# danping/CoSLAM

Measured on AMD Instinct MI355X. Metric: frames/sec for track+local-BA loop, 8 cams 640x480 x 2000 feats (one frame = all 8 cameras), higher is better.
Workload: dtype f32 (KLT, f16 pyramid storage) + f64 (pose, BA)

## Files before the change

### coslam_amd/csrc/cs_common.h

```cpp
#pragma once

#include <hip/hip_fp16.h>
#include <hip/hip_runtime.h>

#include <cstdarg>
#include <cstdint>
#include <cstdio>
#include <cstring>

#include "../../include/coslam_hip.h"

#define CS_MAX_LEVELS 12
#define CS_WAVE 64

void cs_set_error(const char* fmt, ...);
enum { CS_DBG_BA_SYRK = 0, CS_DBG_BA_PACKED = 1, CS_DBG_BA_GRAPHS = 2, CS_DBG_MERGE_PRINT = 3, CS_DBG_COUNT = 4 };
int cs_debug_get(int which);

#define CS_HIP(call)                                                                              \
    do {                                                                                          \
        hipError_t _e = (call);                                                                   \
        if (_e != hipSuccess) {                                                                   \
            cs_set_error("%s failed: %s (%s:%d)", #call, hipGetErrorString(_e), __FILE__, __LINE__); \
            return CS_ERR_HIP;                                                                    \
        }                                                                                         \
    } while (0)

#define CS_CHECK_LAUNCH()                                                                        \
    do {                                                                                         \
        hipError_t _e = hipGetLastError();                                                       \
        if (_e != hipSuccess) {                                                                  \
            cs_set_error("kernel launch failed: %s (%s:%d)", hipGetErrorString(_e), __FILE__, __LINE__); \
            return CS_ERR_HIP;                                                                   \
        }                                                                                        \
    } while (0)

struct CsPyrLayout {
    int W, H, L;
    int w[CS_MAX_LEVELS], h[CS_MAX_LEVELS];
    int64_t off[CS_MAX_LEVELS];
    size_t texels;
};

static inline CsPyrLayout cs_make_layout(int W, int H, int L) {
    CsPyrLayout p;
    memset(&p, 0, sizeof(p));
    p.W = W;
    p.H = H;
    p.L = L;
// ... 82 lines not shown
}

__device__ __forceinline__ double cs_wave_sum_d(double v) {
    v += cs_dpp_d<0xB1, 0xf>(v);
    v += cs_dpp_d<0x4E, 0xf>(v);
    v += cs_dpp_d<0x141, 0xf>(v);
    v += cs_dpp_d<0x140, 0xf>(v);
    v += cs_dpp_d<0x142, 0xa>(v);
    v += cs_dpp_d<0x143, 0xc>(v);
    int lo = __builtin_amdgcn_readlane(__double2loint(v), 63);
    int hi = __builtin_amdgcn_readlane(__double2hiint(v), 63);
    return __hiloint2double(hi, lo);
}

__device__ __forceinline__ int cs_wave_sum_i(int v) {
    v += cs_dpp_i<0xB1, 0xf>(v);
    v += cs_dpp_i<0x4E, 0xf>(v);
    v += cs_dpp_i<0x141, 0xf>(v);
    v += cs_dpp_i<0x140, 0xf>(v);
    v += cs_dpp_i<0x142, 0xa>(v);
    v += cs_dpp_i<0x143, 0xc>(v);
    return __builtin_amdgcn_readlane(v, 63);
}

__device__ __forceinline__ double cs_shfl_xor_d(double v, int d) {
    int lo = __shfl_xor(__double2loint(v), d, 64), hi = __shfl_xor(__double2hiint(v), d, 64);
    return __hiloint2double(hi, lo);
}
__device__ __forceinline__ double cs_readlane_d(double v, int l) {
    int lo = __builtin_amdgcn_readlane(__double2loint(v), l);
    int hi = __builtin_amdgcn_readlane(__double2hiint(v), l);
    return __hiloint2double(hi, lo);
}
template <int M, int DIST>
__device__ __forceinline__ void cs_reduce_step(double* v, int lane) {
    if constexpr (DIST >= 1) {
        constexpr int H = (M + 1) / 2;
        const bool up = (lane & DIST) != 0;
#pragma unroll
        for (int t = 0; t < H; ++t) {
            const double lo = v[t];
            const double hi = (H + t < M) ? v[H + t] : 0.0;
            const double recv = cs_shfl_xor_d(up ? lo : hi, DIST);
            v[t] = (up ? hi : lo) + recv;
        }
        cs_reduce_step<H, DIST / 2>(v, lane);
    }
}
template <int N>
__device__ __forceinline__ void cs_reduce_many(double* v, int lane) {
    cs_reduce_step<N, 32>(v, lane);
}
template <int N>
__host__ __device__ constexpr int cs_reduce_index(int lane) {
    int lo = 0, end = N, m = N;
    for (int d = 32; d >= 1; d >>= 1) {
        const int h = (m + 1) / 2;
        if (lane & d) {
            lo += h;
        } else {
            end = end < lo + h ? end : lo + h;
        }
        m = h;
    }
    return lo < end ? lo : -1;
}
template <int N>
__host__ __device__ constexpr int cs_reduce_owner(int q) {
    for (int l = 0; l < 64; ++l)
        if (cs_reduce_index<N>(l) == q) return l;
    return 0;
}
template <int N>
struct CsOwnerTable {
    int lane[N];
    constexpr CsOwnerTable() : lane{} {
        for (int q = 0; q < N; ++q) lane[q] = cs_reduce_owner<N>(q);
// ... 22 lines not shown
```

### coslam_amd/csrc/klt_seq.hip

```cpp
#include <cstdlib>
#include <mutex>
#include <new>
#include <vector>

#include "klt_internal.h"

static thread_local char g_err[512] = "";
void cs_set_error(const char* fmt, ...) {
    va_list ap;
    va_start(ap, fmt);
    vsnprintf(g_err, sizeof(g_err), fmt, ap);
    va_end(ap);
}

#include <atomic>
static std::atomic<int> g_dbg[CS_DBG_COUNT] = {{-1}, {-1}, {-1}, {-1}};
int cs_debug_get(int which) { return which >= 0 && which < CS_DBG_COUNT ? g_dbg[which].load(std::memory_order_relaxed) : -1; }

extern "C" {

int cs_version(void) { return 100; }
const char* cs_last_error(void) { return g_err; }
int cs_debug_set(const char* key, int value) {
    static const char* names[CS_DBG_COUNT] = {"ba_syrk", "ba_packed", "ba_graphs", "merge_print"};
    for (int k = 0; k < CS_DBG_COUNT; ++k)
        if (key && !strcmp(key, names[k])) {
            g_dbg[k].store(value, std::memory_order_relaxed);
            return CS_OK;
        }
    cs_set_error("cs_debug_set: unknown switch (ba_syrk, ba_packed, ba_graphs, merge_print)");
    return CS_ERR_INVALID;
}


int cs_device_count(void) {
    int n = 0;
    if (hipGetDeviceCount(&n) != hipSuccess) return 0;
    return n;
}

void* cs_stream_create_cu_range(int device, int first_cu, int n_cus) {
    hipDeviceProp_t prop;
    if (hipSetDevice(device) != hipSuccess || hipGetDeviceProperties(&prop, device) != hipSuccess) {
        cs_set_error("cs_stream_create_cu_range: bad device %d", device);
        return nullptr;
    }
    const int total = prop.multiProcessorCount;
    if (first_cu < 0 || n_cus <= 0 || first_cu + n_cus > total) {
        cs_set_error("cs_stream_create_cu_range: range [%d, %d) outside the %d CUs", first_cu, first_cu + n_cus, total);
        return nullptr;
    }
    std::vector<uint32_t> mask((total + 31) / 32, 0u);
    for (int c = first_cu; c < first_cu + n_cus; ++c) mask[c >> 5] |= 1u << (c & 31);
    hipStream_t s = nullptr;
    hipError_t e = hipExtStreamCreateWithCUMask(&s, (uint32_t)mask.size(), mask.data());
    if (e != hipSuccess) {
        cs_set_error("hipExtStreamCreateWithCUMask failed: %s", hipGetErrorString(e));
        return nullptr;
    }
    return (void*)s;
}

void* cs_stream_create_cu_interleaved(int device, int period, int take, int complement) {
// ... 1405 lines not shown
```

### coslam_amd/csrc/poseupdate.hip

```cpp
#include <atomic>
#include <cstdlib>
#include <vector>

#include "cs_common.h"
#include "project_dev.h"
#include "triangulate_dev.h"
#include "history_view.h"
#include "register_rows_dev.h"
#include "small_ops.h"

#pragma clang fp contract(off)

namespace {

constexpr int PU_MAX_CAMS = 16;
constexpr int PU_MAX_HIST = 512;
constexpr int PU_MAX_STORE = 1 << 16;
constexpr int PU_LPS = 8;

struct PuArgs {
    int nCams, N, nMap, cam0, nCamsRun;
    int gateBlocks, dynBlocksPerCam;
    const int* pointFeat;
    const double* R;
// ... 2589 lines not shown
    A.nMap = nMap, A.featRef = (const int4*)d_featRef, A.mapPts = d_mapPts, A.mapCov = d_mapCov, A.sigma = pixelErrVar;
    A.refine = 1, A.select = d_select, A.selectW = d_select;
    return CS_OK;
}
}

extern "C" int cs_feat_ref_advance_refine_dev(cs_track_history* h, void* hip_stream, const cs_poseupdate_cam* cams, int nMap, const int* d_pointFeat,
                                              int curFrame, cs_feat_ref* d_featRef, unsigned char* d_refStatic, int* d_counts, const int* d_list,
                                              int nList, int advanceAll, unsigned char* d_select, int clearSelect, double* d_mapPts,
                                              double* d_mapCov, double pixelErrVar) {
    const char* who = "cs_feat_ref_advance_refine_dev";
    if (!h || !cams || nMap < 1 || nList < 1 || !d_list) {
        cs_set_error("%s: bad arguments", who);
        return CS_ERR_INVALID;
    }
    ArArgs A;
    memset((void*)&A, 0, sizeof(A));
    if (const int rc = ar_fill_refine(who, A, h, cams, nMap, curFrame, d_featRef, d_select, d_mapPts, d_mapCov, pixelErrVar)) return rc;
    if (const int rc = fr_fill(who, A.F, h, cams, nMap, d_pointFeat, curFrame, d_featRef, d_refStatic, d_counts)) return rc;
    A.list = d_list, A.nList = nList, A.advAll = advanceAll ? 1 : 0;
    A.blocksA = ((advanceAll ? nMap : nList) + 255) / 256;
    CS_HIP(hipSetDevice(h->device));
    hipStream_t s = (hipStream_t)hip_stream;
    if (const int rc = hist_alive(h, nMap, s)) return rc;
    A.F.alive = h->alive;
    hist_centres(h, s);
    hipLaunchKernelGGL(k_advance_refine, dim3(A.blocksA + (nList + 3) / 4), dim3(256), 0, s, A);
    if (clearSelect) hipLaunchKernelGGL(k_clear_marks, dim3((nList + 255) / 256), dim3(256), 0, s, d_select, d_list, nList, nMap);
    CS_HIP(hipGetLastError());
    return CS_OK;
}

constexpr int RR_THREADS = 256;
struct RrArgs {
    int nRounds, W, H;
    int* lists;
    int* rvCounts;
    cs_register_pass pass;
    cs_register_cam rcam[RG_MAX_CAMS];
    MgRunCore mg;
    RvArgs rv;
    ArArgs ar;
};
static_assert(sizeof(RrArgs) <= 4096, "k_revisit_rounds: the arguments must fit the kernel-argument segment");
template <int MC>
__global__ __launch_bounds__(RR_THREADS) void k_revisit_rounds(RrArgs A) {
    extern __shared__ double rr_pose[];
    __shared__ MgMiss missList[RR_THREADS / MG_LPC];
    __shared__ int nMiss;
    __shared__ int sCnt[RR_THREADS / 64][5];
    if (rd_ld(A.rvCounts) == 0) return;
    CS_POSE_STREAM_PRIO();
    const int tid = threadIdx.x, lane = tid & 63, wave = tid >> 6, C = A.rv.nCams, cap = A.rv.cap, N = A.rv.N;
    const cs_register_pass& Q = A.pass;
    int cnt[5] = {0, 0, 0, 0, 0};
    for (int r = 0; r < A.nRounds; ++r) {
        const int listed = rd_ld(A.rvCounts + r);
        if (listed == 0) break;
        const int n = listed < cap ? listed : cap;
        const int* list = A.lists + (size_t)r * cap;
        for (int k = wave; k < n * C; k += RR_THREADS / 64) {
            const int row = k / C, c = k - row * C, p = list[row];
            if (p < 0) continue;
            const cs_register_cam& Cm = A.rcam[c];
            const size_t o = (size_t)p * C + c;
            int outSlot = -1, outFlags = 0;
            double m0 = 0, m1 = 0, var[4] = {0, 0, 0, 0}, ivar[4] = {0, 0, 0, 0}, outDist = 0;
            Proj q;
            if (rg_pair_begin(Q, Cm, o, p, A.W, A.H, q, m0, m1, var, ivar, outSlot)) {
                double dMin;
                int iMin;
                rg_pair_scan_wave(Cm, N, lane, m0, m1, ivar, dMin, iMin);
                rg_pair_finish(Q, Cm, p, N, q, m0, m1, dMin, iMin, outSlot, outFlags, outDist);
            }
            if (lane == 0) rg_pair_store(Q, o, outSlot, outFlags, outDist, m0, m1, var);
        }
        __syncthreads();
        const int nB = (n * MG_LPC + RR_THREADS - 1) / RR_THREADS;
        for (int c = 0; c < C; ++c)
            for (int bx = 0; bx < nB; ++bx) {
                mg_running_rows<RR_THREADS>(A.mg, A.ar.cam, list, cap, c, bx, rr_pose, missList, nMiss);
                __syncthreads();
            }
        {
            const bool more = r + 1 < A.nRounds;
            const RvRound Rd{list, A.rvCounts + r, more ? A.lists + (size_t)(r + 1) * cap : nullptr, more ? A.rvCounts + r + 1 : nullptr};
            if (n <= RR_THREADS) {
                rv_decide_rows<MC>(A.rv, Rd);
            } else {
                int* rowCode = (int*)(rr_pose + 12 * (size_t)A.mg.W);
                rv_decide_rows_looped<MC, RR_THREADS>(A.rv, Rd, n, rowCode, rowCode + MC * RV_MAX_ROWS);
            }
        }
        __syncthreads();
        for (int j = tid; j < n; j += RR_THREADS) {
            const int m = list[j];
            if (m >= 0 && m < A.ar.nMap && !A.ar.select[m]) fr_advance_row(A.ar.F, A.ar.cam, m, cnt);
        }
        __syncthreads();
        for (int j = wave; j < n; j += RR_THREADS / 64) {
            const int m = list[j];
            if (m >= 0 && m < A.ar.nMap && A.ar.select[m]) {
                ar_refine_row(A.ar, m, lane, cnt);
                if (lane == 0) A.ar.selectW[m] = 0;
            }
        }
        __syncthreads();
    }
    fr_fold_counts(cnt, sCnt, A.ar.F.counts);
}
template <int MC>
static int rr_dynamic_lds_limit(int device, size_t* out) {
    static std::atomic<long long> last{-1};
    const long long c = last.load(std::memory_order_acquire);
    if (c >= 0 && (int)(c >> 32) == device) {
        *out = (size_t)(c & 0xffffffffll);
// ... 24 lines not shown
    const char* who = "cs_register_revisit_rounds_dev";
    if (!h || !regCams || !cams || !pass) {
        cs_set_error("%s: bad arguments (null history, cameras or pass)", who);
        return CS_ERR_INVALID;
    }
    const int nCams = h->nCams, N = h->N;
    const cs_register_pass& q = *pass;
    if (nCams < 1 || nCams > RG_MAX_CAMS || nCams > RD_MAX_CAMS || N < 1 || W < 1 || H < 1 || !(q.maxDist > 0) || !(q.sigmaSearch >= 0) ||
        !(q.sigmaMerge >= 0) || (q.mapFlags && !(q.maxDistDynamic > 0))) {
        cs_set_error("%s: bad arguments (1..%d cameras, N >= 1, maxDist > 0; mapFlags with maxDistDynamic > 0)", who, RD_MAX_CAMS);
        return CS_ERR_INVALID;
    }
    if (!q.M || !q.cov || !q.pointFeat || !q.slot || !q.m || !q.var || !q.dist || !q.flags || q.M != d_mapPts || q.cov != d_mapCov ||
        q.pointFeat != d_pointFeat) {
        cs_set_error("%s: the pass needs every table, and its map, covariances and feature table are the ones refined", who);
        return CS_ERR_INVALID;
    }
    if (nMap < 1 || cap < 1 || cap > RV_MAX_ROWS || nRounds < 1 || nRounds > 8 || kinds < 1 || kinds > 3 || mapBase < 0 || !(tolPix >= 0) ||
        !d_rvLists || !d_rvCounts || (long long)nCams * N > RD_FEAT || (long long)nCams * nMap * nCams > 0x7fffffffLL) {
        cs_set_error("%s: bad arguments (1..%d rows, 1..8 rounds, kinds 1..3, the rounds' lists and counts)", who, RV_MAX_ROWS);
        return CS_ERR_INVALID;
    }
    RrArgs A;
    memset((void*)&A, 0, sizeof(A));
    for (int c = 0; c < nCams; ++c) {
        const cs_register_cam& rc = regCams[c];
        if (!rc.K || !rc.R || !rc.t || !rc.xy || !rc.state || !rc.slot2map) {
            cs_set_error("%s: null pointer in search camera %d", who, c);
            return CS_ERR_INVALID;
        }
        A.rcam[c] = rc;
    }
    A.nRounds = nRounds, A.W = W, A.H = H, A.lists = d_rvLists, A.rvCounts = d_rvCounts;
    A.pass = q;
    A.pass.P = cap, A.pass.list = nullptr;
    if (const int rc = ar_fill_refine(who, A.ar, h, cams, nMap, curFrame, d_featRef, d_regOut, d_mapPts, d_mapCov, pixelErrVar)) return rc;
    if (const int rc = fr_fill(who, A.ar.F, h, cams, nMap, d_pointFeat, curFrame, d_featRef, d_refStatic, d_frefCounts)) return rc;
    if (const int rc = mg_fill_running(who, A.mg, h, cams, 0, nMap, d_mapPts, d_mapCov, q.slot, q.flags, pixelErrVar, tolPix, d_mergeCache,
                                       d_mergeable, nullptr))
        return rc;
    if (const int rc = rv_fill(who, A.rv, nCams, N, nMap, cap, mapBase, kinds, d_nextLoop, d_visitLoop, q.slot, q.flags, d_mergeable, d_mapFlags,
                               d_pointFeat, d_slot2map, d_attached, d_regOut, d_decideScratch, d_curList, d_curCount, curCap, d_rvCnt,
                               d_rvCounts + nRounds))
        return rc;
    CS_HIP(hipSetDevice(h->device));
    hipStream_t s = (hipStream_t)hip_stream;
    const int MC = nCams <= 8 ? 8 : RD_MAX_CAMS;
    const size_t lds = sizeof(double) * 12 * (size_t)A.mg.W + (cap > RR_THREADS ? sizeof(int) * (size_t)(MC + 1) * RV_MAX_ROWS : 0);
    size_t ldsMax = 0;
    if (const int rc = MC == 8 ? rr_dynamic_lds_limit<8>(h->device, &ldsMax) : rr_dynamic_lds_limit<RD_MAX_CAMS>(h->device, &ldsMax)) return rc;
    if (lds > ldsMax) {
        cs_set_error("%s: %zu B of LDS (a history window of %d frames, lists of %d rows, %d cameras) where the launch may carry %zu", who, lds,
                     A.mg.W, cap, nCams, ldsMax);
        return CS_ERR_INVALID;
    }
    if (const int rc = hist_alive(h, nMap, s)) return rc;
    A.ar.F.alive = h->alive;
    hist_centres(h, s);
    if (MC == 8)
        hipLaunchKernelGGL(k_revisit_rounds<8>, dim3(1), dim3(RR_THREADS), lds, s, A);
    else
        hipLaunchKernelGGL(k_revisit_rounds<RD_MAX_CAMS>, dim3(1), dim3(RR_THREADS), lds, s, A);
    CS_HIP(hipGetLastError());
    return CS_OK;
}

extern "C" int cs_track_history_segments(const cs_track_history* h, cs_feat_seg** d_pool, int* cap, int** d_count) {
    if (!h) {
        cs_set_error("cs_track_history_segments: null handle");
        return CS_ERR_INVALID;
    }
    if (d_pool) *d_pool = (cs_feat_seg*)h->segPool;
    if (cap) *cap = h->segCap;
    if (d_count) *d_count = h->segCount;
    return CS_OK;
}

extern "C" int cs_track_history_segment_counts(const cs_track_history* h, int* counts) {
    if (!h || !counts) {
        cs_set_error("cs_track_history_segment_counts: bad arguments");
        return CS_ERR_INVALID;
    }
    CS_HIP(hipSetDevice(h->device));
    CS_HIP(hipMemcpy(counts, h->segCount, sizeof(int) * h->nCams, hipMemcpyDeviceToHost));
    return CS_OK;
}

extern "C" int cs_track_history_load_segments(cs_track_history* h, const cs_feat_seg* segs, int n) {
    if (!h || n < 0 || n > h->segCap || (n > 0 && !segs)) {
        cs_set_error("cs_track_history_load_segments: bad arguments (at most %d segments per camera)", h ? h->segCap : 0);
        return CS_ERR_INVALID;
    }
    CS_HIP(hipSetDevice(h->device));
    std::vector<int> cnt(h->nCams, n);
    for (int c = 0; c < h->nCams && n > 0; ++c)
// ... 308 lines not shown
```

### coslam_amd/csrc/pose.hip

```cpp
#include "cs_common.h"

#pragma clang fp contract(off)

namespace {

constexpr int WS_LDS_MAX = 4096;
constexpr int SMALL_NPTS = 64;

__device__ __forceinline__ void so3_exp(const double w[3], double R[9]) {
    double theta = sqrt(w[0] * w[0] + w[1] * w[1] + w[2] * w[2]);
    if (theta == 0) {
        R[0] = 1, R[1] = 0, R[2] = 0, R[3] = 0, R[4] = 1, R[5] = 0, R[6] = 0, R[7] = 0, R[8] = 1;
        return;
    }
    double hw0 = w[0] / theta, hw1 = w[1] / theta, hw2 = w[2] / theta;
    double st, ct;
    if (theta < 0.5) {
        const double x2 = theta * theta;
        double ps = 1.0 / 355687428096000.0;
        ps = ps * x2 - 1.0 / 1307674368000.0;
        ps = ps * x2 + 1.0 / 6227020800.0;
        ps = ps * x2 - 1.0 / 39916800.0;
        ps = ps * x2 + 1.0 / 362880.0;
        ps = ps * x2 - 1.0 / 5040.0;
        ps = ps * x2 + 1.0 / 120.0;
        ps = ps * x2 - 1.0 / 6.0;
        st = theta + theta * (x2 * ps);
        double pc = 1.0 / 20922789888000.0;
        pc = pc * x2 - 1.0 / 87178291200.0;
        pc = pc * x2 + 1.0 / 479001600.0;
        pc = pc * x2 - 1.0 / 3628800.0;
        pc = pc * x2 + 1.0 / 40320.0;
        pc = pc * x2 - 1.0 / 720.0;
        pc = pc * x2 + 1.0 / 24.0;
        const double c = 1.0 - (0.5 * x2 - x2 * x2 * pc);
        ct = 1 - c;
    } else {
        st = sin(theta);
        ct = 1 - cos(theta);
    }
    double hw0hw0 = hw0 * hw0, hw0hw1 = hw0 * hw1, hw0hw2 = hw0 * hw2;
    double hw1hw1 = hw1 * hw1, hw1hw2 = hw1 * hw2, hw2hw2 = hw2 * hw2;
    R[0] = -ct * hw1hw1 - ct * hw2hw2 + 1;
    R[1] = ct * hw0hw1 - st * hw2;
    R[2] = st * hw1 + ct * hw0hw2;
    R[3] = st * hw2 + ct * hw0hw1;
    R[4] = -ct * hw0hw0 - ct * hw2hw2 + 1;
    R[5] = ct * hw1hw2 - st * hw0;
    R[6] = ct * hw0hw2 - st * hw1;
    R[7] = st * hw0 + ct * hw1hw2;
    R[8] = -ct * hw0hw0 - ct * hw1hw1 + 1;
}

__device__ __forceinline__ void mat33AB(const double* A, const double* B, double* C) {
    double T[9];
#pragma unroll
    for (int i = 0; i < 3; ++i)
#pragma unroll
        for (int j = 0; j < 3; ++j) T[3 * i + j] = A[3 * i] * B[j] + A[3 * i + 1] * B[3 + j] + A[3 * i + 2] * B[6 + j];
#pragma unroll
    for (int i = 0; i < 9; ++i) C[i] = T[i];
}

__device__ __forceinline__ void project(const double* K, const double* R, const double* t, const double* M, double* m) {
    double X = R[0] * M[0] + R[1] * M[1] + R[2] * M[2] + t[0];
    double Y = R[3] * M[0] + R[4] * M[1] + R[5] * M[2] + t[1];
    double Z = R[6] * M[0] + R[7] * M[1] + R[8] * M[2] + t[2];
    double u = K[0] * X + K[1] * Y + K[2] * Z;
    double v = K[3] * X + K[4] * Y + K[5] * Z;
    double w = K[6] * X + K[7] * Y + K[8] * Z;
    m[0] = u / w;
    m[1] = v / w;
}

__device__ __forceinline__ double cs_shfl_d(double v, int srcLane) {
    int lo = __shfl(__double2loint(v), srcLane, 64), hi = __shfl(__double2hiint(v), srcLane, 64);
    return __hiloint2double(hi, lo);
}
__device__ __forceinline__ void solve66_lanes(double m, int lane, double* param) {
    const int r = lane / 7, j = lane - 7 * r;
    const bool in = r < 6;
#pragma unroll
    for (int c = 0; c < 6; ++c) {
        double best = fabs(cs_readlane_d(m, 7 * c + c));
        int p = c;
#pragma unroll
        for (int rr = c + 1; rr < 6; ++rr) {
            const double v = fabs(cs_readlane_d(m, 7 * rr + c));
            if (v > best) best = v, p = rr;
        }
        const int srcRow = r == c ? p : (r == p ? c : r);
        const double sw = cs_shfl_d(m, in ? 7 * srcRow + j : lane);
        m = sw;
        const double d = cs_readlane_d(m, 7 * c + c);
        const double q = m / d;
        if (r == c && j > c) m = q;
        const double f = cs_shfl_d(m, in ? 7 * r + c : lane);
        const double pr = cs_shfl_d(m, in ? 7 * c + j : lane);
        const double e = m - f * pr;
        if (in && r != c && j > c) m = e;
    }
#pragma unroll
    for (int rr = 0; rr < 6; ++rr) param[rr] = cs_readlane_d(m, 7 * rr + 6);
}

__device__ __forceinline__ double tukey(double e, double tau) {
    if (e >= tau) return 0;
    e /= tau;
    e = 1 - e * e;
    return e * e;
}

struct PoseCtx {
    const double* K;
    const double* Ms;
    const double* ms;
    double* Ws;
    int npts;
    double* red;
    double pM[3], pm[2];
    double dR[3][9];
    int myEntry;
};

constexpr int NSUM = 28;
__device__ __forceinline__ int solve_entry_of_lane(int lane) {
    const int r = lane / 7, j = lane - 7 * r;
    if (r >= 6) return 27;
    if (j == 6) return 21 + r;
    const int a = r < j ? r : j, b = r < j ? j : r;
    return a * 6 - (a * (a - 1)) / 2 + (b - a);
}
template <int PB>
__device__ __forceinline__ void block_sum28(double (&v)[NSUM], double* lds , int& par, int myEntry, double& mine,
                                            double& err) {
    constexpr int NW = PB / 64;
    const int lane = threadIdx.x & 63, wv = threadIdx.x >> 6;
    cs_reduce_many<NSUM>(v, lane);
    if (NW == 1) {
        constexpr CsOwnerTable<NSUM> T{};
        int owner = 0;
#pragma unroll
        for (int q = 0; q < NSUM; ++q) owner = myEntry == q ? T.lane[q] : owner;
        mine = cs_shfl_d(v[0], owner);
        err = cs_readlane_d(v[0], T.lane[27]);
        return;
    }
    const int have = cs_reduce_index<NSUM>(lane);
    double* buf = lds + par * (NW * NSUM);
    par ^= 1;
    if (have >= 0) buf[wv * NSUM + have] = v[0];
    __syncthreads();
    double s = buf[myEntry], e = buf[27];
#pragma unroll
    for (int w = 1; w < NW; ++w) s += buf[w * NSUM + myEntry], e += buf[w * NSUM + 27];
    mine = s, err = e;
}

template <int PB>
__device__ void lm_pass(const PoseCtx& c, const double* R, const double* t, bool reweight, double tau, int& par, double& mine, double& err) {
    const double eps = 1e-8;
    const double ieps = 1e8;
    double R1[3][9];
#pragma unroll
    for (int a = 0; a < 3; ++a) mat33AB(R, c.dR[a], R1[a]);
    double acc[NSUM];
#pragma unroll
    for (int q = 0; q < NSUM; ++q) acc[q] = 0;
    for (int i = threadIdx.x; i < c.npts; i += PB) {
        double pM[3], pm[2];
        if (i < PB) {
            pM[0] = c.pM[0], pM[1] = c.pM[1], pM[2] = c.pM[2], pm[0] = c.pm[0], pm[1] = c.pm[1];
        } else {
            pM[0] = c.Ms[3 * i], pM[1] = c.Ms[3 * i + 1], pM[2] = c.Ms[3 * i + 2], pm[0] = c.ms[2 * i], pm[1] = c.ms[2 * i + 1];
        }
        double rm0[2], rm[2], J[12];
        project(c.K, R, t, pM, rm0);
        const double dx = rm0[0] - pm[0], dy = rm0[1] - pm[1];
        double w;
        if (reweight) {
            w = tukey(sqrt(dx * dx + dy * dy), tau);
            c.Ws[i] = w;
        } else {
            w = c.Ws[i];
        }
        acc[27] += (dx * dx + dy * dy) * w;
#pragma unroll
        for (int a = 0; a < 3; ++a) {
            project(c.K, R1[a], t, pM, rm);
            J[a] = (rm[0] - rm0[0]) * ieps;
            J[6 + a] = (rm[1] - rm0[1]) * ieps;
        }
#pragma unroll
        for (int a = 0; a < 3; ++a) {
            double t1[3] = {t[0], t[1], t[2]};
            t1[a] = t[a] + eps;
            project(c.K, R, t1, pM, rm);
            J[3 + a] = (rm[0] - rm0[0]) * ieps;
            J[9 + a] = (rm[1] - rm0[1]) * ieps;
        }
#pragma unroll
        for (int q = 0; q < 12; ++q) J[q] = w * J[q];
        const double r0 = (-rm0[0] + pm[0]) * w, r1 = (-rm0[1] + pm[1]) * w;
        int q = 0;
#pragma unroll
        for (int r = 0; r < 6; ++r)
#pragma unroll
            for (int cc = r; cc < 6; ++cc) acc[q++] += J[r] * J[cc] + J[6 + r] * J[6 + cc];
#pragma unroll
        for (int r = 0; r < 6; ++r) acc[21 + r] += J[r] * r0 + J[6 + r] * r1;
    }
    block_sum28<PB>(acc, c.red, par, c.myEntry, mine, err);
}

__device__ __forceinline__ void lm_solve(double mine, double lambda, double* param) {
    const int lane = threadIdx.x & 63, r = lane / 7, j = lane - 7 * r;
    solve66_lanes(r == j ? mine + lambda : mine, lane, param);
}

__device__ __forceinline__ void update_pose(const double* R, const double* t, const double* p, double* Rn, double* tn) {
    double dR[9];
    so3_exp(p, dR);
    mat33AB(R, dR, Rn);
    tn[0] = t[0] + p[3];
    tn[1] = t[1] + p[4];
    tn[2] = t[2] + p[5];
}

template <int PB>
__device__ bool weighted_lm(const PoseCtx& c, const double* R0, const double* t0, double* R_opt, double* t_opt,
                            cs_pose_option& opt, bool reweight, double tau, int& par) {
    double param[6];
    double ne, cand, err;
    opt.npts = c.npts;
    opt.lambda = opt.lambda0;
    lm_pass<PB>(c, R0, t0, reweight, tau, par, ne, err);
    opt.err0 = err;
    opt.err = opt.err0;
    double R[9], t[3], R_tmp[9], t_tmp[3];
#pragma unroll
    for (int i = 0; i < 9; ++i) R[i] = R_tmp[i] = R0[i];
#pragma unroll
    for (int i = 0; i < 3; ++i) t[i] = t_tmp[i] = t0[i];
    opt.retTypeLM = 1;
    int i = 0;
    for (; i < opt.maxIterLM; ++i) {
        lm_solve(ne, opt.lambda, param);
        update_pose(R, t, param, R_opt, t_opt);
        double p2 = param[0] * param[0] + param[1] * param[1] + param[2] * param[2] + param[3] * param[3] +
                    param[4] * param[4] + param[5] * param[5];
        if (p2 < opt.epsParamChangeLM) {
            opt.retTypeLM = 0;
            break;
        }
        lm_pass<PB>(c, R_opt, t_opt, false, tau, par, cand, err);
        if (fabs(err - opt.err) < opt.epsErrorChangeLM) {
            opt.retTypeLM = 0;
            break;
        }
        if (err <= opt.err) {
#pragma unroll
            for (int q = 0; q < 9; ++q) R[q] = R_tmp[q] = R_opt[q];
#pragma unroll
            for (int q = 0; q < 3; ++q) t[q] = t_tmp[q] = t_opt[q];
            ne = cand;
            opt.err = err;
            opt.lambda /= 10;
        } else {
            opt.lambda *= 10;
            if (opt.lambda > 1e+18) {
                opt.retTypeLM = -1;
                break;
            }
        }
    }
    if (opt.retTypeLM == -1) {
#pragma unroll
        for (int q = 0; q < 9; ++q) R_opt[q] = R_tmp[q];
#pragma unroll
        for (int q = 0; q < 3; ++q) t_opt[q] = t_tmp[q];
    }
    opt.err = err;
    opt.nIterLM = i;
    opt.verboseRW += i < opt.maxIterLM ? i + 1 : i;
    return opt.retTypeLM >= 0;
}

#if defined(CS_IC_NUM_VGPR)
#define CS_IC_ATTR __attribute__((amdgpu_num_vgpr(CS_IC_NUM_VGPR)))
#elif defined(CS_IC_WAVES_PER_EU)
#define CS_IC_ATTR __attribute__((amdgpu_waves_per_eu(CS_IC_WAVES_PER_EU, CS_IC_WAVES_PER_EU)))
#else
#define CS_IC_ATTR
#endif
template <int PB>
__global__ __launch_bounds__(PB) CS_IC_ATTR void k_intracam(int ptsStride, const double* __restrict__ Kall,
                                                 const double* __restrict__ R0all, const double* __restrict__ t0all,
                                                 const int* __restrict__ nptsAll, const double* __restrict__ prevErrs,
                                                 const double* __restrict__ MsAll, const double* __restrict__ msAll,
                                                 double tau, double* __restrict__ RoptAll, double* __restrict__ toptAll,
                                                 cs_pose_option* __restrict__ optAll, int* __restrict__ okAll,
                                                 double* __restrict__ wsScratch) {
    extern __shared__ __attribute__((aligned(16))) double smem[];
    CS_POSE_STREAM_PRIO();
    const int pb = blockIdx.x;
    constexpr int NW = PB / 64;
    double* red = smem;
    double* sK = smem + 2 * NW * NSUM;
    double* WsL = sK + 12;
    const int npts = nptsAll[pb];
    if (threadIdx.x < 9) sK[threadIdx.x] = Kall[9 * pb + threadIdx.x];
    PoseCtx c;
    c.K = sK;
    c.Ms = MsAll + (size_t)3 * ptsStride * pb;
    c.ms = msAll + (size_t)2 * ptsStride * pb;
    c.npts = npts;
    c.red = red;
    c.myEntry = solve_entry_of_lane(threadIdx.x & 63);
    c.Ws = wsScratch ? (wsScratch + (size_t)ptsStride * pb) : WsL;
#pragma unroll
    for (int a = 0; a < 3; ++a) {
        double w[3] = {0, 0, 0};
        w[a] = 1e-8;
        so3_exp(w, c.dR[a]);
    }
    if ((int)threadIdx.x < npts) {
        const int i = threadIdx.x;
        c.pM[0] = c.Ms[3 * i], c.pM[1] = c.Ms[3 * i + 1], c.pM[2] = c.Ms[3 * i + 2], c.pm[0] = c.ms[2 * i], c.pm[1] = c.ms[2 * i + 1];
    } else {
        c.pM[0] = c.pM[1] = c.pM[2] = c.pm[0] = c.pm[1] = 0;
    }
    for (int i = threadIdx.x; i < npts; i += PB)
        c.Ws[i] = prevErrs ? tukey(fabs(prevErrs[(size_t)ptsStride * pb + i]), tau) : 1.0;
    __syncthreads();

    cs_pose_option opt = optAll[pb];
    double R[9], t[3], R_opt[9], t_opt[3];
#pragma unroll
    for (int i = 0; i < 9; ++i) R[i] = R_opt[i] = R0all[9 * pb + i];
#pragma unroll
    for (int i = 0; i < 3; ++i) t[i] = t_opt[i] = t0all[3 * pb + i];
    bool ret = true;
    int k = 0, par = 0;
    opt.errRW = -1;
    opt.verboseRW = 0;
    for (; k < opt.maxIterRW; ++k) {
        if (!weighted_lm<PB>(c, R, t, R_opt, t_opt, opt, k > 0, tau, par)) {
            ret = false;
            break;
        }
        opt.lambda0 = opt.lambda;
        if (opt.errRW < 0) {
            opt.errRW = opt.err;
        } else {
            if (fabs(opt.err - opt.errRW) < opt.epsErrorChangeRW) {
                ret = true;
                break;
            }
// ... 148 lines not shown
```

Baseline: 2079.

## Spread first revisit round across a multi-block grid with last-block ticket handoff

```diff
diff --git a/coslam_amd/csrc/cs_common.h b/coslam_amd/csrc/cs_common.h
--- a/coslam_amd/csrc/cs_common.h
+++ b/coslam_amd/csrc/cs_common.h
@@ -14,7 +14,7 @@
 #define CS_WAVE 64
 
 void cs_set_error(const char* fmt, ...);
-enum { CS_DBG_BA_SYRK = 0, CS_DBG_BA_PACKED = 1, CS_DBG_BA_GRAPHS = 2, CS_DBG_MERGE_PRINT = 3, CS_DBG_COUNT = 4 };
+enum { CS_DBG_BA_SYRK = 0, CS_DBG_BA_PACKED = 1, CS_DBG_BA_GRAPHS = 2, CS_DBG_MERGE_PRINT = 3, CS_DBG_REVISIT_GRID = 4, CS_DBG_COUNT = 5 };
 int cs_debug_get(int which);
 
 #define CS_HIP(call)                                                                              \
diff --git a/coslam_amd/csrc/klt_seq.hip b/coslam_amd/csrc/klt_seq.hip
--- a/coslam_amd/csrc/klt_seq.hip
+++ b/coslam_amd/csrc/klt_seq.hip
@@ -14,7 +14,7 @@
 }
 
 #include <atomic>
-static std::atomic<int> g_dbg[CS_DBG_COUNT] = {{-1}, {-1}, {-1}, {-1}};
+static std::atomic<int> g_dbg[CS_DBG_COUNT] = {{-1}, {-1}, {-1}, {-1}, {-1}};
 int cs_debug_get(int which) { return which >= 0 && which < CS_DBG_COUNT ? g_dbg[which].load(std::memory_order_relaxed) : -1; }
 
 extern "C" {
@@ -22,13 +22,13 @@
 int cs_version(void) { return 100; }
 const char* cs_last_error(void) { return g_err; }
 int cs_debug_set(const char* key, int value) {
-    static const char* names[CS_DBG_COUNT] = {"ba_syrk", "ba_packed", "ba_graphs", "merge_print"};
+    static const char* names[CS_DBG_COUNT] = {"ba_syrk", "ba_packed", "ba_graphs", "merge_print", "revisit_grid"};
     for (int k = 0; k < CS_DBG_COUNT; ++k)
         if (key && !strcmp(key, names[k])) {
             g_dbg[k].store(value, std::memory_order_relaxed);
             return CS_OK;
         }
-    cs_set_error("cs_debug_set: unknown switch (ba_syrk, ba_packed, ba_graphs, merge_print)");
+    cs_set_error("cs_debug_set: unknown switch (ba_syrk, ba_packed, ba_graphs, merge_print, revisit_grid)");
     return CS_ERR_INVALID;
 }
 
diff --git a/coslam_amd/csrc/poseupdate.hip b/coslam_amd/csrc/poseupdate.hip
--- a/coslam_amd/csrc/poseupdate.hip
+++ b/coslam_amd/csrc/poseupdate.hip
@@ -2645,10 +2645,15 @@
 }
 
 constexpr int RR_THREADS = 256;
+constexpr int RR_UNIT_ROWS = RR_THREADS / MG_LPC;
+constexpr int RR_GRID_PER_CAM = 2;
+constexpr int RR_TICKET_WORD = 2;
+static_assert(RR_TICKET_WORD < RD_SCRATCH_HEAD, "k_revisit_rounds: the ticket lives in the decision scratch's head");
 struct RrArgs {
     int nRounds, W, H;
     int* lists;
     int* rvCounts;
+    int* ticket;
     cs_register_pass pass;
     cs_register_cam rcam[RG_MAX_CAMS];
     MgRunCore mg;
@@ -2656,45 +2661,78 @@
     ArArgs ar;
 };
 static_assert(sizeof(RrArgs) <= 4096, "k_revisit_rounds: the arguments must fit the kernel-argument segment");
+__device__ __forceinline__ void rr_search_pair(const RrArgs& A, int p, int c, int lane) {
+    const cs_register_pass& Q = A.pass;
+    const cs_register_cam& Cm = A.rcam[c];
+    const int N = A.rv.N;
+    const size_t o = (size_t)p * A.rv.nCams + c;
+    int outSlot = -1, outFlags = 0;
+    double m0 = 0, m1 = 0, var[4] = {0, 0, 0, 0}, ivar[4] = {0, 0, 0, 0}, outDist = 0;
+    Proj q;
+    if (rg_pair_begin(Q, Cm, o, p, A.W, A.H, q, m0, m1, var, ivar, outSlot)) {
+        double dMin;
+        int iMin;
+        rg_pair_scan_wave(Cm, N, lane, m0, m1, ivar, dMin, iMin);
+        rg_pair_finish(Q, Cm, p, N, q, m0, m1, dMin, iMin, outSlot, outFlags, outDist);
+    }
+    if (lane == 0) rg_pair_store(Q, o, outSlot, outFlags, outDist, m0, m1, var);
+}
 template <int MC>
 __global__ __launch_bounds__(RR_THREADS) void k_revisit_rounds(RrArgs A) {
     extern __shared__ double rr_pose[];
     __shared__ MgMiss missList[RR_THREADS / MG_LPC];
     __shared__ int nMiss;
     __shared__ int sCnt[RR_THREADS / 64][5];
-    if (rd_ld(A.rvCounts) == 0) return;
+    __shared__ int sLast;
+    const int listed0 = rd_ld(A.rvCounts);
+    if (listed0 == 0) return;
     CS_POSE_STREAM_PRIO();
-    const int tid = threadIdx.x, lane = tid & 63, wave = tid >> 6, C = A.rv.nCams, cap = A.rv.cap, N = A.rv.N;
-    const cs_register_pass& Q = A.pass;
+    const int tid = threadIdx.x, lane = tid & 63, wave = tid >> 6, C = A.rv.nCams, cap = A.rv.cap;
+    {
+        const int n = listed0 < cap ? listed0 : cap;
+        const int nB = (n + RR_UNIT_ROWS - 1) / RR_UNIT_ROWS, nU = C * nB;
+        const int* list = A.lists;
+        for (int u = blockIdx.x; u < nU; u += gridDim.x) {
+            const int c = u / nB, bx = u - c * nB, j1 = min(n, (bx + 1) * RR_UNIT_ROWS);
+            for (int j = bx * RR_UNIT_ROWS + wave; j < j1; j += RR_THREADS / 64) {
+                const int p = list[j];
+                if (p >= 0) rr_search_pair(A, p, c, lane);
+            }
+            __syncthreads();
+            mg_running_rows<RR_THREADS>(A.mg, A.ar.cam, list, cap, c, bx, rr_pose, missList, nMiss);
+            __syncthreads();
+        }
+        asm volatile("s_waitcnt vmcnt(0)" ::: "memory");
+        __syncthreads();
+        if (tid == 0) {
+            if ((int)blockIdx.x < nU) __builtin_amdgcn_fence(__ATOMIC_RELEASE, "agent");
+            sLast = __hip_atomic_fetch_add(A.ticket, 1, __ATOMIC_RELAXED, __HIP_MEMORY_SCOPE_AGENT) == (int)gridDim.x - 1;
+        }
+        __syncthreads();
+        if (!sLast) return;
+        __builtin_amdgcn_fence(__ATOMIC_ACQUIRE, "agent");
+        if (tid == 0) rd_st(A.ticket, 0);
+        __syncthreads();
+    }
     int cnt[5] = {0, 0, 0, 0, 0};
     for (int r = 0; r < A.nRounds; ++r) {
-        const int listed = rd_ld(A.rvCounts + r);
+        const int listed = r == 0 ? listed0 : rd_ld(A.rvCounts + r);
         if (listed == 0) break;
         const int n = listed < cap ? listed : cap;
         const int* list = A.lists + (size_t)r * cap;
-        for (int k = wave; k < n * C; k += RR_THREADS / 64) {
-            const int row = k / C, c = k - row * C, p = list[row];
-            if (p < 0) continue;
-            const cs_register_cam& Cm = A.rcam[c];
-            const size_t o = (size_t)p * C + c;
-            int outSlot = -1, outFlags = 0;
-            double m0 = 0, m1 = 0, var[4] = {0, 0, 0, 0}, ivar[4] = {0, 0, 0, 0}, outDist = 0;
-            Proj q;
-            if (rg_pair_begin(Q, Cm, o, p, A.W, A.H, q, m0, m1, var, ivar, outSlot)) {
-                double dMin;
-                int iMin;
-                rg_pair_scan_wave(Cm, N, lane, m0, m1, ivar, dMin, iMin);
-                rg_pair_finish(Q, Cm, p, N, q, m0, m1, dMin, iMin, outSlot, outFlags, outDist);
+        if (r > 0) {
+            for (int k = wave; k < n * C; k += RR_THREADS / 64) {
+                const int row = k / C, c = k - row * C, p = list[row];
+                if (p >= 0) rr_search_pair(A, p, c, lane);
             }
-            if (lane == 0) rg_pair_store(Q, o, outSlot, outFlags, outDist, m0, m1, var);
-        }
-        __syncthreads();
-        const int nB = (n * MG_LPC + RR_THREADS - 1) / RR_THREADS;
-        for (int c = 0; c < C; ++c)
-            for (int bx = 0; bx < nB; ++bx) {
-                mg_running_rows<RR_THREADS>(A.mg, A.ar.cam, list, cap, c, bx, rr_pose, missList, nMiss);
-                __syncthreads();
-            }
+            __syncthreads();
+            const int nB = (n + RR_UNIT_ROWS - 1) / RR_UNIT_ROWS;
+            for (int c = 0; c < C; ++c)
+                for (int bx = 0; bx < nB; ++bx) {
+                    mg_running_rows<RR_THREADS>(A.mg, A.ar.cam, list, cap, c, bx, rr_pose, missList, nMiss);
+                    __syncthreads();
+                }
+        }
         {
             const bool more = r + 1 < A.nRounds;
             const RvRound Rd{list, A.rvCounts + r, more ? A.lists + (size_t)(r + 1) * cap : nullptr, more ? A.rvCounts + r + 1 : nullptr};
@@ -2785,6 +2823,7 @@
         A.rcam[c] = rc;
     }
     A.nRounds = nRounds, A.W = W, A.H = H, A.lists = d_rvLists, A.rvCounts = d_rvCounts;
+    A.ticket = (int*)d_decideScratch + RR_TICKET_WORD;
     A.pass = q;
     A.pass.P = cap, A.pass.list = nullptr;
     if (const int rc = ar_fill_refine(who, A.ar, h, cams, nMap, curFrame, d_featRef, d_regOut, d_mapPts, d_mapCov, pixelErrVar)) return rc;
@@ -2810,10 +2849,12 @@
     if (const int rc = hist_alive(h, nMap, s)) return rc;
     A.ar.F.alive = h->alive;
     hist_centres(h, s);
+    const int nUnits = nCams * ((cap + RR_UNIT_ROWS - 1) / RR_UNIT_ROWS), forced = cs_debug_get(CS_DBG_REVISIT_GRID);
+    const int grid = forced >= 1 ? (forced < 65535 ? forced : 65535) : (nUnits < RR_GRID_PER_CAM * nCams ? nUnits : RR_GRID_PER_CAM * nCams);
     if (MC == 8)
-        hipLaunchKernelGGL(k_revisit_rounds<8>, dim3(1), dim3(RR_THREADS), lds, s, A);
+        hipLaunchKernelGGL(k_revisit_rounds<8>, dim3(grid), dim3(RR_THREADS), lds, s, A);
     else
-        hipLaunchKernelGGL(k_revisit_rounds<RD_MAX_CAMS>, dim3(1), dim3(RR_THREADS), lds, s, A);
+        hipLaunchKernelGGL(k_revisit_rounds<RD_MAX_CAMS>, dim3(grid), dim3(RR_THREADS), lds, s, A);
     CS_HIP(hipGetLastError());
     return CS_OK;
 }
```

After: 2078. Within noise of the previous version (-0.1%).

## Rework pose LM solve to column-per-lane layout with DPP/permlane reductions

Applied to the files above, without the earlier changes.

```diff
diff --git a/coslam_amd/csrc/cs_common.h b/coslam_amd/csrc/cs_common.h
--- a/coslam_amd/csrc/cs_common.h
+++ b/coslam_amd/csrc/cs_common.h
@@ -163,6 +163,28 @@
     int hi = __builtin_amdgcn_readlane(__double2hiint(v), l);
     return __hiloint2double(hi, lo);
 }
+template <int DIST>
+__device__ __forceinline__ double cs_swap_add_d(double x, double y) {
+    const unsigned xl = (unsigned)__double2loint(x), xh = (unsigned)__double2hiint(x);
+    const unsigned yl = (unsigned)__double2loint(y), yh = (unsigned)__double2hiint(y);
+    if constexpr (DIST == 32) {
+        const auto l = __builtin_amdgcn_permlane32_swap(xl, yl, false, false);
+        const auto h = __builtin_amdgcn_permlane32_swap(xh, yh, false, false);
+        return __hiloint2double((int)h[0], (int)l[0]) + __hiloint2double((int)h[1], (int)l[1]);
+    } else {
+        const auto l = __builtin_amdgcn_permlane16_swap(xl, yl, false, false);
+        const auto h = __builtin_amdgcn_permlane16_swap(xh, yh, false, false);
+        return __hiloint2double((int)h[0], (int)l[0]) + __hiloint2double((int)h[1], (int)l[1]);
+    }
+}
+template <int DIST>
+__device__ __forceinline__ double cs_dpp_xor_d(double v) {
+    static_assert(DIST == 8 || DIST == 4 || DIST == 2 || DIST == 1, "a distance inside a 16-lane row");
+    if constexpr (DIST == 8) return cs_dpp_d<0x128, 0xf>(v);
+    else if constexpr (DIST == 4) return cs_dpp_d<0x141, 0xf>(cs_dpp_d<0x1B, 0xf>(v));
+    else if constexpr (DIST == 2) return cs_dpp_d<0x4E, 0xf>(v);
+    else return cs_dpp_d<0xB1, 0xf>(v);
+}
 template <int M, int DIST>
 __device__ __forceinline__ void cs_reduce_step(double* v, int lane) {
     if constexpr (DIST >= 1) {
@@ -172,8 +194,12 @@
         for (int t = 0; t < H; ++t) {
             const double lo = v[t];
             const double hi = (H + t < M) ? v[H + t] : 0.0;
-            const double recv = cs_shfl_xor_d(up ? lo : hi, DIST);
-            v[t] = (up ? hi : lo) + recv;
+            if constexpr (DIST >= 16) {
+                v[t] = cs_swap_add_d<DIST>(lo, hi);
+            } else {
+                const double recv = cs_dpp_xor_d<DIST>(up ? lo : hi);
+                v[t] = (up ? hi : lo) + recv;
+            }
         }
         cs_reduce_step<H, DIST / 2>(v, lane);
     }
diff --git a/coslam_amd/csrc/pose.hip b/coslam_amd/csrc/pose.hip
--- a/coslam_amd/csrc/pose.hip
+++ b/coslam_amd/csrc/pose.hip
@@ -1,4 +1,6 @@
 #include "cs_common.h"
+#include "pose_math.h"
+#include "pose_solve_dev.h"
 
 #pragma clang fp contract(off)
 
@@ -6,61 +8,6 @@
 
 constexpr int WS_LDS_MAX = 4096;
 constexpr int SMALL_NPTS = 64;
-
-__device__ __forceinline__ void so3_exp(const double w[3], double R[9]) {
-    double theta = sqrt(w[0] * w[0] + w[1] * w[1] + w[2] * w[2]);
-    if (theta == 0) {
-        R[0] = 1, R[1] = 0, R[2] = 0, R[3] = 0, R[4] = 1, R[5] = 0, R[6] = 0, R[7] = 0, R[8] = 1;
-        return;
-    }
-    double hw0 = w[0] / theta, hw1 = w[1] / theta, hw2 = w[2] / theta;
-    double st, ct;
-    if (theta < 0.5) {
-        const double x2 = theta * theta;
-        double ps = 1.0 / 355687428096000.0;
-        ps = ps * x2 - 1.0 / 1307674368000.0;
-        ps = ps * x2 + 1.0 / 6227020800.0;
-        ps = ps * x2 - 1.0 / 39916800.0;
-        ps = ps * x2 + 1.0 / 362880.0;
-        ps = ps * x2 - 1.0 / 5040.0;
-        ps = ps * x2 + 1.0 / 120.0;
-        ps = ps * x2 - 1.0 / 6.0;
-        st = theta + theta * (x2 * ps);
-        double pc = 1.0 / 20922789888000.0;
-        pc = pc * x2 - 1.0 / 87178291200.0;
-        pc = pc * x2 + 1.0 / 479001600.0;
-        pc = pc * x2 - 1.0 / 3628800.0;
-        pc = pc * x2 + 1.0 / 40320.0;
-        pc = pc * x2 - 1.0 / 720.0;
-        pc = pc * x2 + 1.0 / 24.0;
-        const double c = 1.0 - (0.5 * x2 - x2 * x2 * pc);
-        ct = 1 - c;
-    } else {
-        st = sin(theta);
-        ct = 1 - cos(theta);
-    }
-    double hw0hw0 = hw0 * hw0, hw0hw1 = hw0 * hw1, hw0hw2 = hw0 * hw2;
-    double hw1hw1 = hw1 * hw1, hw1hw2 = hw1 * hw2, hw2hw2 = hw2 * hw2;
-    R[0] = -ct * hw1hw1 - ct * hw2hw2 + 1;
-    R[1] = ct * hw0hw1 - st * hw2;
-    R[2] = st * hw1 + ct * hw0hw2;
-    R[3] = st * hw2 + ct * hw0hw1;
-    R[4] = -ct * hw0hw0 - ct * hw2hw2 + 1;
-    R[5] = ct * hw1hw2 - st * hw0;
-    R[6] = ct * hw0hw2 - st * hw1;
-    R[7] = st * hw0 + ct * hw1hw2;
-    R[8] = -ct * hw0hw0 - ct * hw1hw1 + 1;
-}
-
-__device__ __forceinline__ void mat33AB(const double* A, const double* B, double* C) {
-    double T[9];
-#pragma unroll
-    for (int i = 0; i < 3; ++i)
-#pragma unroll
-        for (int j = 0; j < 3; ++j) T[3 * i + j] = A[3 * i] * B[j] + A[3 * i + 1] * B[3 + j] + A[3 * i + 2] * B[6 + j];
-#pragma unroll
-    for (int i = 0; i < 9; ++i) C[i] = T[i];
-}
 
 __device__ __forceinline__ void project(const double* K, const double* R, const double* t, const double* M, double* m) {
     double X = R[0] * M[0] + R[1] * M[1] + R[2] * M[2] + t[0];
@@ -73,37 +20,6 @@
     m[1] = v / w;
 }
 
-__device__ __forceinline__ double cs_shfl_d(double v, int srcLane) {
-    int lo = __shfl(__double2loint(v), srcLane, 64), hi = __shfl(__double2hiint(v), srcLane, 64);
-    return __hiloint2double(hi, lo);
-}
-__device__ __forceinline__ void solve66_lanes(double m, int lane, double* param) {
-    const int r = lane / 7, j = lane - 7 * r;
-    const bool in = r < 6;
-#pragma unroll
-    for (int c = 0; c < 6; ++c) {
-        double best = fabs(cs_readlane_d(m, 7 * c + c));
-        int p = c;
-#pragma unroll
-        for (int rr = c + 1; rr < 6; ++rr) {
-            const double v = fabs(cs_readlane_d(m, 7 * rr + c));
-            if (v > best) best = v, p = rr;
-        }
-        const int srcRow = r == c ? p : (r == p ? c : r);
-        const double sw = cs_shfl_d(m, in ? 7 * srcRow + j : lane);
-        m = sw;
-        const double d = cs_readlane_d(m, 7 * c + c);
-        const double q = m / d;
-        if (r == c && j > c) m = q;
-        const double f = cs_shfl_d(m, in ? 7 * r + c : lane);
-        const double pr = cs_shfl_d(m, in ? 7 * c + j : lane);
-        const double e = m - f * pr;
-        if (in && r != c && j > c) m = e;
-    }
-#pragma unroll
-    for (int rr = 0; rr < 6; ++rr) param[rr] = cs_readlane_d(m, 7 * rr + 6);
-}
-
 __device__ __forceinline__ double tukey(double e, double tau) {
     if (e >= tau) return 0;
     e /= tau;
@@ -119,51 +35,41 @@
     int npts;
     double* red;
     double pM[3], pm[2];
-    double dR[3][9];
-    int myEntry;
+    int myEntry[6];
 };
 
 constexpr int NSUM = 28;
-__device__ __forceinline__ int solve_entry_of_lane(int lane) {
-    const int r = lane / 7, j = lane - 7 * r;
-    if (r >= 6) return 27;
-    if (j == 6) return 21 + r;
-    const int a = r < j ? r : j, b = r < j ? j : r;
-    return a * 6 - (a * (a - 1)) / 2 + (b - a);
-}
 template <int PB>
-__device__ __forceinline__ void block_sum28(double (&v)[NSUM], double* lds , int& par, int myEntry, double& mine,
-                                            double& err) {
+__device__ __forceinline__ void block_sum28(double (&v)[NSUM], double* lds , int& par, const int (&myEntry)[6],
+                                            double (&mine)[6], double& err) {
     constexpr int NW = PB / 64;
     const int lane = threadIdx.x & 63, wv = threadIdx.x >> 6;
     cs_reduce_many<NSUM>(v, lane);
-    if (NW == 1) {
-        constexpr CsOwnerTable<NSUM> T{};
-        int owner = 0;
-#pragma unroll
-        for (int q = 0; q < NSUM; ++q) owner = myEntry == q ? T.lane[q] : owner;
-        mine = cs_shfl_d(v[0], owner);
-        err = cs_readlane_d(v[0], T.lane[27]);
-        return;
-    }
     const int have = cs_reduce_index<NSUM>(lane);
     double* buf = lds + par * (NW * NSUM);
     par ^= 1;
     if (have >= 0) buf[wv * NSUM + have] = v[0];
     __syncthreads();
-    double s = buf[myEntry], e = buf[27];
-#pragma unroll
-    for (int w = 1; w < NW; ++w) s += buf[w * NSUM + myEntry], e += buf[w * NSUM + 27];
-    mine = s, err = e;
+    double e = buf[27];
+#pragma unroll
+    for (int r = 0; r < 6; ++r) mine[r] = buf[myEntry[r]];
+#pragma unroll
+    for (int w = 1; w < NW; ++w) {
+#pragma unroll
+        for (int r = 0; r < 6; ++r) mine[r] += buf[w * NSUM + myEntry[r]];
+        e += buf[w * NSUM + 27];
+    }
+    err = e;
 }
 
 template <int PB>
-__device__ void lm_pass(const PoseCtx& c, const double* R, const double* t, bool reweight, double tau, int& par, double& mine, double& err) {
+__device__ void lm_pass(const PoseCtx& c, const double* R, const double* t, bool reweight, double tau, int& par, double (&mine)[6], double& err) {
     const double eps = 1e-8;
     const double ieps = 1e8;
     double R1[3][9];
-#pragma unroll
-    for (int a = 0; a < 3; ++a) mat33AB(R, c.dR[a], R1[a]);
+    mat33_perturbed<0>(R, R1[0]);
+    mat33_perturbed<1>(R, R1[1]);
+    mat33_perturbed<2>(R, R1[2]);
     double acc[NSUM];
 #pragma unroll
     for (int q = 0; q < NSUM; ++q) acc[q] = 0;
@@ -213,9 +119,12 @@
     block_sum28<PB>(acc, c.red, par, c.myEntry, mine, err);
 }
 
-__device__ __forceinline__ void lm_solve(double mine, double lambda, double* param) {
-    const int lane = threadIdx.x & 63, r = lane / 7, j = lane - 7 * r;
-    solve66_lanes(r == j ? mine + lambda : mine, lane, param);
+__device__ __forceinline__ void lm_solve(const double (&mine)[6], double lambda, double* param) {
+    const int lane = threadIdx.x & 63;
+    double col[6];
+#pragma unroll
+    for (int r = 0; r < 6; ++r) col[r] = r == lane ? mine[r] + lambda : mine[r];
+    solve66_lanes(col, lane, param);
 }
 
 __device__ __forceinline__ void update_pose(const double* R, const double* t, const double* p, double* Rn, double* tn) {
@@ -231,7 +140,7 @@
 __device__ bool weighted_lm(const PoseCtx& c, const double* R0, const double* t0, double* R_opt, double* t_opt,
                             cs_pose_option& opt, bool reweight, double tau, int& par) {
     double param[6];
-    double ne, cand, err;
+    double ne[6], cand[6], err;
     opt.npts = c.npts;
     opt.lambda = opt.lambda0;
     lm_pass<PB>(c, R0, t0, reweight, tau, par, ne, err);
@@ -263,7 +172,8 @@
             for (int q = 0; q < 9; ++q) R[q] = R_tmp[q] = R_opt[q];
 #pragma unroll
             for (int q = 0; q < 3; ++q) t[q] = t_tmp[q] = t_opt[q];
-            ne = cand;
+#pragma unroll
+            for (int q = 0; q < 6; ++q) ne[q] = cand[q];
             opt.err = err;
             opt.lambda /= 10;
         } else {
@@ -316,14 +226,9 @@
     c.ms = msAll + (size_t)2 * ptsStride * pb;
     c.npts = npts;
     c.red = red;
-    c.myEntry = solve_entry_of_lane(threadIdx.x & 63);
+#pragma unroll
+    for (int r = 0; r < 6; ++r) c.myEntry[r] = solve66_entry(r, min((int)(threadIdx.x & 63), 6));
     c.Ws = wsScratch ? (wsScratch + (size_t)ptsStride * pb) : WsL;
-#pragma unroll
-    for (int a = 0; a < 3; ++a) {
-        double w[3] = {0, 0, 0};
-        w[a] = 1e-8;
-        so3_exp(w, c.dR[a]);
-    }
     if ((int)threadIdx.x < npts) {
         const int i = threadIdx.x;
         c.pM[0] = c.Ms[3 * i], c.pM[1] = c.Ms[3 * i + 1], c.pM[2] = c.Ms[3 * i + 2], c.pm[0] = c.ms[2 * i], c.pm[1] = c.ms[2 * i + 1];
diff --git a/coslam_amd/csrc/pose_math.h b/coslam_amd/csrc/pose_math.h
--- /dev/null
+++ b/coslam_amd/csrc/pose_math.h
@@ -0,0 +1,83 @@
+#pragma once
+
+#include <cmath>
+
+#if defined(__clang__)
+#pragma clang fp contract(off)
+#endif
+
+#if defined(__HIPCC__)
+#define CS_PM_FN static __host__ __device__ __forceinline__
+#define CS_PM_UNROLL _Pragma("unroll")
+#else
+#define CS_PM_FN static inline
+#define CS_PM_UNROLL
+#endif
+
+CS_PM_FN void so3_exp(const double w[3], double R[9]) {
+    double theta = sqrt(w[0] * w[0] + w[1] * w[1] + w[2] * w[2]);
+    if (theta == 0) {
+        R[0] = 1, R[1] = 0, R[2] = 0, R[3] = 0, R[4] = 1, R[5] = 0, R[6] = 0, R[7] = 0, R[8] = 1;
+        return;
+    }
+    double hw0 = w[0] / theta, hw1 = w[1] / theta, hw2 = w[2] / theta;
+    double st, ct;
+    if (theta < 0.5) {
+        const double x2 = theta * theta;
+        double ps = 1.0 / 355687428096000.0;
+        ps = ps * x2 - 1.0 / 1307674368000.0;
+        ps = ps * x2 + 1.0 / 6227020800.0;
+        ps = ps * x2 - 1.0 / 39916800.0;
+        ps = ps * x2 + 1.0 / 362880.0;
+        ps = ps * x2 - 1.0 / 5040.0;
+        ps = ps * x2 + 1.0 / 120.0;
+        ps = ps * x2 - 1.0 / 6.0;
+        st = theta + theta * (x2 * ps);
+        double pc = 1.0 / 20922789888000.0;
+        pc = pc * x2 - 1.0 / 87178291200.0;
+        pc = pc * x2 + 1.0 / 479001600.0;
+        pc = pc * x2 - 1.0 / 3628800.0;
+        pc = pc * x2 + 1.0 / 40320.0;
+        pc = pc * x2 - 1.0 / 720.0;
+        pc = pc * x2 + 1.0 / 24.0;
+        const double c = 1.0 - (0.5 * x2 - x2 * x2 * pc);
+        ct = 1 - c;
+    } else {
+        st = sin(theta);
+        ct = 1 - cos(theta);
+    }
+    double hw0hw0 = hw0 * hw0, hw0hw1 = hw0 * hw1, hw0hw2 = hw0 * hw2;
+    double hw1hw1 = hw1 * hw1, hw1hw2 = hw1 * hw2, hw2hw2 = hw2 * hw2;
+    R[0] = -ct * hw1hw1 - ct * hw2hw2 + 1;
+    R[1] = ct * hw0hw1 - st * hw2;
+    R[2] = st * hw1 + ct * hw0hw2;
+    R[3] = st * hw2 + ct * hw0hw1;
+    R[4] = -ct * hw0hw0 - ct * hw2hw2 + 1;
+    R[5] = ct * hw1hw2 - st * hw0;
+    R[6] = ct * hw0hw2 - st * hw1;
+    R[7] = st * hw0 + ct * hw1hw2;
+    R[8] = -ct * hw0hw0 - ct * hw1hw1 + 1;
+}
+
+CS_PM_FN void mat33AB(const double* A, const double* B, double* C) {
+    double T[9];
+    CS_PM_UNROLL
+    for (int i = 0; i < 3; ++i)
+        CS_PM_UNROLL
+        for (int j = 0; j < 3; ++j) T[3 * i + j] = A[3 * i] * B[j] + A[3 * i + 1] * B[3 + j] + A[3 * i + 2] * B[6 + j];
+    CS_PM_UNROLL
+    for (int i = 0; i < 9; ++i) C[i] = T[i];
+}
+
+template <int K>
+CS_PM_FN void mat33_perturbed(const double* R, double* C) {
+    constexpr int P = (K + 1) % 3, Q = (K + 2) % 3;
+    const double eps = 1e-8;
+    CS_PM_UNROLL
+    for (int i = 0; i < 3; ++i) {
+        const double rp = R[3 * i + P], rq = R[3 * i + Q];
+        C[3 * i + K] = R[3 * i + K];
+        C[3 * i + P] = rp + rq * eps;
+        C[3 * i + Q] = rp * (-eps) + rq;
+    }
+}
diff --git a/coslam_amd/csrc/pose_solve_dev.h b/coslam_amd/csrc/pose_solve_dev.h
--- /dev/null
+++ b/coslam_amd/csrc/pose_solve_dev.h
@@ -0,0 +1,49 @@
+#pragma once
+
+#include "cs_common.h"
+
+#pragma clang fp contract(off)
+
+#ifdef __HIPCC__
+
+__device__ __forceinline__ int solve66_entry(int r, int j) {
+    if (j >= 6) return 21 + r;
+    const int a = r < j ? r : j, b = r < j ? j : r;
+    return a * 6 - (a * (a - 1)) / 2 + (b - a);
+}
+__device__ __forceinline__ void solve66_lanes(double (&col)[6], int lane, double* param) {
+    const int j = lane;
+#pragma unroll
+    for (int c = 0; c < 6; ++c) {
+        double best = fabs(col[c]);
+        int p = c;
+#pragma unroll
+        for (int rr = c + 1; rr < 6; ++rr) {
+            const double v = fabs(col[rr]);
+            if (v > best) best = v, p = rr;
+        }
+        p = __builtin_amdgcn_readlane(p, c);
+#pragma unroll
+        for (int rr = c + 1; rr < 6; ++rr) {
+            const double a = col[c], b = col[rr];
+            col[c] = p == rr ? b : a;
+            col[rr] = p == rr ? a : b;
+        }
+        const double d = cs_readlane_d(col[c], c);
+        double f[6];
+#pragma unroll
+        for (int rr = 0; rr < 6; ++rr) f[rr] = cs_readlane_d(col[rr], c);
+        const double q = col[c] / d;
+        if (j > c) col[c] = q;
+#pragma unroll
+        for (int rr = 0; rr < 6; ++rr) {
+            if (rr == c) continue;
+            const double e = col[rr] - f[rr] * col[c];
+            if (j > c) col[rr] = e;
+        }
+    }
+#pragma unroll
+    for (int rr = 0; rr < 6; ++rr) param[rr] = cs_readlane_d(col[rr], 6);
+}
+
+#endif
```

Result: faster. 2077 before, 2143 after (median of 6 runs) (+3.2%).
